# charlesq34/pointnet2

Measured on AMD Instinct MI355X. Metric: point-clouds/sec for SA(FPS+ball+group) B=32 N=4096→1024 nsample=32, higher is better.
Workload: dtype f32

## Files before the change

pointnet2_amd/csrc/fps_batch_body.h:

```cpp
#pragma once
#include "fps_pruned_body.h"

namespace pn2 {

constexpr int kBtCand = PN2_WAVE;
constexpr int kBtMaxW = 8;
#ifndef PN2_BT_UT
#define PN2_BT_UT 512
#endif
constexpr int kBtUT = PN2_BT_UT;
constexpr int kBtT = kBtUT + PN2_WAVE;
constexpr unsigned kBtEnd = 0x100u, kBtFill = 0x200u, kBtCountMask = 0xffu;

struct BtXchg {
    double list[kBtCand];
    unsigned cnt[kBtMaxW];
    unsigned bound[kBtMaxW];
    unsigned count;
    unsigned single;
    unsigned theta, vlast;
    unsigned pad[4];
};
static_assert(sizeof(BtXchg) % 16 == 0, "16-byte rows");

__host__ __device__ constexpr size_t fps_batch_xchg_offset(int P, int UT = kBtUT) { return (fps_pruned_lds_bytes(P, UT) + 15) & ~(size_t)15; }
__host__ __device__ constexpr size_t fps_batch_lds_bytes(int P, int UT = kBtUT) { return fps_batch_xchg_offset(P, UT) + 2 * sizeof(BtXchg) + 16 * kBtCand; }

__device__ __forceinline__ float vmax_f32(float a, float b)
{
    float r;
    asm("v_max_f32 %0, %1, %2" : "=v"(r) : "v"(a), "v"(b));
    return r;
}
__device__ __forceinline__ float vmed3_f32(float a, float b, float c)
{
    float r;
    asm("v_med3_f32 %0, %1, %2, %3" : "=v"(r) : "v"(a), "v"(b), "v"(c));
    return r;
}

__device__ __forceinline__ int bt_wave_max_i32_lane63(int v)
{
#define PN2_BT_STEP(ctrl) v = max(v, __builtin_amdgcn_update_dpp(0, v, ctrl, 0xf, 0xf, true))
    PN2_BT_STEP(0xB1);
    PN2_BT_STEP(0x4E);
    PN2_BT_STEP(0x141);
    PN2_BT_STEP(0x140);
    PN2_BT_STEP(0x142);
    PN2_BT_STEP(0x143);
#undef PN2_BT_STEP
    return v;
}

__device__ __forceinline__ void lds_max_u32(unsigned *p, unsigned v)
{
    asm volatile("ds_max_u32 %0, %1" :: "v"((unsigned)(size_t)p), "v"(v) : "memory");
}

inline bool fps_batch_covers(int ranks) { return ranks > 512 && ranks <= 8192; }
#ifdef PN2_BT_LAB_NEVER_AUTO
inline bool fps_batch_pays(int, int) { return false; }
#else
inline bool fps_batch_pays(int ranks, int m) { return fps_batch_covers(ranks) && m >= 256; }
#endif

#ifdef PN2_BT_STATS
__device__ unsigned long long g_bt_stats[16];
#ifndef PN2_BT_STATS_FROM
#define PN2_BT_STATS_FROM 0
#endif
#define PN2_BT_STAT(i, v) do { if (lane == 0 && cloud == 0 && j >= PN2_BT_STATS_FROM) atomicAdd(&g_bt_stats[i], (unsigned long long)(v)); } while (0)
#define PN2_BT_CLOCK() __builtin_readcyclecounter()
#else
#define PN2_BT_STAT(i, v) do { } while (0)
#define PN2_BT_CLOCK() 0ll
#pragma clang diagnostic ignored "-Wunused-variable"
#endif

#ifndef PN2_BT_LIST_HI
#define PN2_BT_LIST_HI 36
#define PN2_BT_LIST_LO 20
#endif
#ifndef PN2_BT_EARLY
#define PN2_BT_EARLY 48
#endif
#ifndef PN2_BT_ASM_LOOP
#define PN2_BT_ASM_LOOP 1
#endif
#ifndef PN2_BT_G0
#define PN2_BT_G0 0.10f
#endif
#ifndef PN2_BT_PACKED_FROM
#define PN2_BT_PACKED_FROM 16
#endif
#ifndef PN2_BT_SLOW_MIN
#define PN2_BT_SLOW_MIN 3
#define PN2_BT_QUICK 1
#define PN2_BT_SINGLE0 16
#define PN2_BT_SINGLE1 512
#endif

template <int P, int GS, bool PUBLISH, int UT = kBtUT>
__device__ __forceinline__ void fps_batch_body(int n, int m, int Q, int cloud, const float *__restrict__ xyz,
                                               int *__restrict__ out, float *__restrict__ out_xyz,
                                               unsigned long long *__restrict__ tagged, char *smem, unsigned tag = 1u)
{
    constexpr int W = UT / PN2_WAVE, NS = UT * P;
    constexpr int GW = P / GS;
    constexpr int CAP = kBtCand / W;
    constexpr int BT = UT + PN2_WAVE;
    static_assert((W * GW == 32 && (W == 4 || W == 8)) || (W == 8 && (GW == 2 || GW == 1)),
                  "32 groups on four or eight updater waves; 16 / 8 groups (2048 / 1024 rank slots) on eight");
    float4 *lds_rank = reinterpret_cast<float4 *>(smem + 256);
    BtXchg *xch = reinterpret_cast<BtXchg *>(smem + fps_batch_xchg_offset(P, UT));
    float4 *ring = reinterpret_cast<float4 *>(smem + fps_batch_xchg_offset(P, UT) + 2 * sizeof(BtXchg));

    const float *__restrict__ src = xyz + (size_t)cloud * n * 3;
    int *__restrict__ dst = out + (size_t)cloud * m;
    float *__restrict__ dxyz = out_xyz ? out_xyz + (size_t)cloud * m * 3 : nullptr;
    pn2_gu64 *gtag = PUBLISH ? (pn2_gu64 *)(tagged + (size_t)cloud * m) : nullptr;
    const int t = threadIdx.x;
    const int lane = t & 63;
    const int w = __builtin_amdgcn_readfirstlane(t >> 6);

    int j = 1;
    const int jE = min(PN2_BT_EARLY, m);
    int fill_k = -1;

    if (w == W) {
#ifndef PN2_NO_SETPRIO
        __builtin_amdgcn_s_setprio(3);
#endif
        for (int i = lane; i < (int)(2 * sizeof(BtXchg) / 4); i += PN2_WAVE) reinterpret_cast<unsigned *>(xch)[i] = 0u;
        for (int i = 0; i < kPrPrologueBarriers; ++i) __syncthreads();
        long long e0 = 0;
        for (; j < jE; ++j) {
            if (j == 8) e0 = (long long)__builtin_readcyclecounter();
            __syncthreads();
        }
        const float round_cyc = jE >= 24 ? (float)((long long)__builtin_readcyclecounter() - e0) / (float)(jE - 8) : 1e30f;
        float bt_cyc = 0.f, bt_smp = 0.f;
        int bt_n = 0, bt_paid = 0, run = PN2_BT_SINGLE0, a_prev = 0, single_next = 0;
        long long qb = 0;
        float g = PN2_BT_G0;
        int par = 0;
        if (j < m)
        for (;;) {
            const long long q0 = PN2_BT_CLOCK();
            {
                const long long qn = (long long)__builtin_readcyclecounter();
                if (bt_n > 0) {
                    bt_cyc = 0.75f * bt_cyc + (float)(qn - qb); bt_smp = 0.75f * bt_smp + (float)a_prev;
                    if (bt_n > PN2_BT_QUICK) {
                        if (bt_cyc > bt_smp * round_cyc * (bt_n > PN2_BT_SLOW_MIN ? 1.0f : 1.5f)) {
                            single_next = run;
                            run = min(2 * run, PN2_BT_SINGLE1);
                            bt_n = -1; bt_paid = 0; bt_cyc = 0.f; bt_smp = 0.f;
                        } else if (++bt_paid >= 8) {
                            run = PN2_BT_SINGLE0;
                        }
                    }
                }
                qb = qn;
                ++bt_n;
            }
            __syncthreads();
            const long long q1 = PN2_BT_CLOCK();
            BtXchg &X = xch[par];
            if (lane == 0) __hip_atomic_store(&xch[par ^ 1].count, 0u, __ATOMIC_RELAXED, __HIP_MEMORY_SCOPE_WORKGROUP);
            const uint4 c4 = *reinterpret_cast<const uint4 *>(X.cnt), c5 = *reinterpret_cast<const uint4 *>(X.cnt + 4);
            const uint4 b4 = *reinterpret_cast<const uint4 *>(X.bound), b5 = *reinterpret_cast<const uint4 *>(X.bound + 4);
            const double key = X.list[lane];
            const unsigned cw = X.cnt[lane / CAP];
            const bool valid = (unsigned)(lane & (CAP - 1)) < cw;
            const unsigned lowc = valid ? (unsigned)__double2loint(key) : 0u;
            typedef float bt_f4 __attribute__((ext_vector_type(4)));
            const bt_f4 cand = *reinterpret_cast<const bt_f4 *>(&lds_rank[lowc]);
            const int boundb = __builtin_amdgcn_readfirstlane((int)max(max(max(b4.x, b4.y), max(b4.z, b4.w)), max(max(b5.x, b5.y), max(b5.z, b5.w))));
            const int total = __builtin_amdgcn_readfirstlane((int)(c4.x + c4.y + c4.z + c4.w + c5.x + c5.y + c5.z + c5.w));
            int cval = valid ? __double2hiint(key) : (int)0xBF800000;
            const int clo = (int)lowc;
            int a = 0;
            int vlastb = 0;
            bool fill = false;
            const unsigned ring_base = (unsigned)(size_t)ring, count_addr = (unsigned)(size_t)&X.count;
            const long long q2 = PN2_BT_CLOCK();
            int bh;
            unsigned long long eq;
            auto argmax = [&]() __attribute__((always_inline)) {
                bh = __builtin_amdgcn_readlane(bt_wave_max_i32_lane63(cval), 63);
                eq = __ballot(cval == bh);
                if (__popcll(eq) != 1) {
                    PN2_BT_STAT(11, 1);
                    const double kq = cval == bh ? __hiloint2double(cval, clo) : -1.0;
                    const double km = wave_max_f64_lane63(kq);
                    const int ml = __builtin_amdgcn_readlane(__double2loint(km), 63);
                    eq = __ballot(cval == bh && clo == ml);
                    eq &= 0ull - eq;
                }
            };
            argmax();
            const int amax = min(m - j, kBtCand);
            unsigned raddr = ring_base, na = 1u;
#if PN2_BT_ASM_LOOP
            const float cx = cand.x, cy = cand.y, cz = cand.z;
            for (;;) {
                int reason, t_wl, t_sx, t_sy, t_sz, t_ms, t_cnt;
                int v_t;
                float v_dx, v_dy, v_dz;
                asm volatile(
                    "s_branch 1f\n\t"
                    "0:\n\t"
                    "s_mov_b32 %[bh], %[ms]\n\t"
                    "1:\n\t"
                    "s_mov_b64 exec, %[eq]\n\t"
                    "ds_write_b128 %[raddr], %[cand]\n\t"
                    "ds_write_b32 %[caddr], %[na]\n\t"
                    "v_mov_b32 %[cval], 0xbf800000\n\t"
                    "s_mov_b64 exec, -1\n\t"
                    "s_ff1_i32_b64 %[wl], %[eq]\n\t"
                    "s_add_i32 %[a], %[a], 1\n\t"
                    "v_add_u32 %[raddr], 16, %[raddr]\n\t"
                    "v_add_u32 %[na], 1, %[na]\n\t"
                    "s_cmp_ge_i32 %[a], %[amax]\n\t"
                    "s_cbranch_scc1 2f\n\t"
                    "v_readlane_b32 %[sx], %[cx], %[wl]\n\t"
                    "v_readlane_b32 %[sy], %[cy], %[wl]\n\t"
                    "v_max_i32_dpp %[t], %[cval], %[cval] quad_perm:[1,0,3,2] row_mask:0xf bank_mask:0xf bound_ctrl:0\n\t"
                    "v_readlane_b32 %[sz], %[cz], %[wl]\n\t"
                    "v_subrev_f32 %[dx], %[sx], %[cx]\n\t"
                    "v_max_i32_dpp %[t], %[t], %[t] quad_perm:[2,3,0,1] row_mask:0xf bank_mask:0xf bound_ctrl:0\n\t"
                    "v_subrev_f32 %[dy], %[sy], %[cy]\n\t"
                    "v_subrev_f32 %[dz], %[sz], %[cz]\n\t"
                    "v_max_i32_dpp %[t], %[t], %[t] row_half_mirror row_mask:0xf bank_mask:0xf bound_ctrl:0\n\t"
                    "v_mul_f32 %[dx], %[dx], %[dx]\n\t"
                    "v_mul_f32 %[dy], %[dy], %[dy]\n\t"
                    "v_max_i32_dpp %[t], %[t], %[t] row_mirror row_mask:0xf bank_mask:0xf bound_ctrl:0\n\t"
                    "v_mul_f32 %[dz], %[dz], %[dz]\n\t"
                    "v_add_f32 %[dx], %[dx], %[dy]\n\t"
                    "v_max_i32_dpp %[t], %[t], %[t] row_bcast:15 row_mask:0xf bank_mask:0xf bound_ctrl:0\n\t"
                    "v_add_f32 %[dx], %[dx], %[dz]\n\t"
                    "s_nop 0\n\t"
                    "v_max_i32_dpp %[t], %[t], %[t] row_bcast:31 row_mask:0xf bank_mask:0xf bound_ctrl:0\n\t"
                    "v_min_f32 %[cval], %[dx], %[cval]\n\t"
                    "s_nop 0\n\t"
                    "v_readlane_b32 %[ms], %[t], 63\n\t"
                    "s_nop 0\n\t"
                    "s_cmp_lt_i32 %[ms], %[bound]\n\t"
                    "s_cbranch_scc1 3f\n\t"
                    "v_cmp_eq_u32_e64 %[eq], %[ms], %[cval]\n\t"
                    "s_bcnt1_i32_b64 %[cnt], %[eq]\n\t"
                    "s_cmp_eq_u32 %[cnt], 1\n\t"
                    "s_cbranch_scc1 0b\n\t"
                    "s_mov_b32 %[reason], 2\n\t"
                    "s_branch 4f\n\t"
                    "2:\n\t"
                    "s_mov_b32 %[reason], 0\n\t"
                    "s_branch 4f\n\t"
                    "3:\n\t"
                    "s_mov_b32 %[reason], 1\n\t"
                    "4:"
                    : [cval] "+v"(cval), [raddr] "+v"(raddr), [na] "+v"(na), [eq] "+s"(eq), [a] "+s"(a), [bh] "+s"(bh),
                      [reason] "=&s"(reason), [wl] "=&s"(t_wl), [sx] "=&s"(t_sx), [sy] "=&s"(t_sy), [sz] "=&s"(t_sz), [ms] "=&s"(t_ms), [cnt] "=&s"(t_cnt),
                      [t] "=&v"(v_t), [dx] "=&v"(v_dx), [dy] "=&v"(v_dy), [dz] "=&v"(v_dz)
                    : [cand] "v"(cand), [caddr] "v"(count_addr), [cx] "v"(cx), [cy] "v"(cy), [cz] "v"(cz), [amax] "s"(amax), [bound] "s"(boundb)
                    : "memory", "scc");
                vlastb = bh;
                if (reason != 2) break;
                PN2_BT_STAT(12, 1);
                argmax();
                if (bh < boundb) break;
            }
#else
            for (;;) {
                asm volatile("s_mov_b64 exec, %1\n\t"
                             "ds_write_b128 %2, %3\n\t"
                             "ds_write_b32 %4, %5\n\t"
                             "v_mov_b32 %0, 0xbf800000\n\t"
                             "s_mov_b64 exec, -1"
                             : "+v"(cval) : "s"(eq), "v"(raddr), "v"(cand), "v"(count_addr), "v"(na) : "memory");
                const int wl = (int)__builtin_ctzll(eq);
                raddr += 16u; na += 1u;
                a = __builtin_amdgcn_readfirstlane(a + 1);
                vlastb = bh;
                if (a >= amax) break;
                const int ms = __builtin_amdgcn_readlane(bt_wave_max_i32_lane63(cval), 63);
                const float sx = __int_as_float(__builtin_amdgcn_readlane(__float_as_int(cand.x), wl));
                const float sy = __int_as_float(__builtin_amdgcn_readlane(__float_as_int(cand.y), wl));
                const float sz = __int_as_float(__builtin_amdgcn_readlane(__float_as_int(cand.z), wl));
                const float d = sqdist(cand.x, cand.y, cand.z, sx, sy, sz);
                cval = __float_as_int(vmin_f32(d, __int_as_float(cval)));
                if (ms < boundb) break;
                eq = __ballot(cval == ms);
                bh = ms;
                if (__popcll(eq) != 1) {
                    PN2_BT_STAT(12, 1);
                    argmax();
                    if (bh < boundb) break;
                }
            }
#endif
            if (vlastb == 0) { fill = true; fill_k = __builtin_amdgcn_readlane(__float_as_int(cand.w), (int)__builtin_ctzll(eq)); }
            const long long q3 = PN2_BT_CLOCK();
            if (total > PN2_BT_LIST_HI) g = fmaxf(g * 0.8f, 1.0f / 128.0f);
            else if (total < PN2_BT_LIST_LO) g = fminf(g * 1.25f, 0.5f);
            X.theta = __float_as_uint(__fmul_rn(__int_as_float(vlastb), 1.0f - g));
            X.vlast = (unsigned)vlastb;
            a_prev = a;
            int single = min(single_next, m - (j + a));
            if (single_next) { PN2_BT_STAT(13, single); PN2_BT_STAT(14, 1); }
            single_next = 0;
            single = __builtin_amdgcn_readfirstlane(single);
            X.single = (unsigned)single;
            if (lane == 0)
                __hip_atomic_store(&X.count, (unsigned)a | kBtEnd | (fill ? kBtFill : 0u), __ATOMIC_RELEASE, __HIP_MEMORY_SCOPE_WORKGROUP);
            PN2_BT_STAT(0, 1); PN2_BT_STAT(1, a); PN2_BT_STAT(4, total); PN2_BT_STAT(6, q2 - q1); PN2_BT_STAT(7, q3 - q2); PN2_BT_STAT(8, q1 - q0);
            j = __builtin_amdgcn_readfirstlane(j + a);
            if (fill || j >= m) break;
            for (int i = 0; i < single; ++i) __syncthreads();
            j += single;
            if (j >= m) break;
            par ^= 1;
        }
    } else {
        PrSlots<P> S;
        fps_pruned_prologue<P, GS, UT>(n, Q, src, smem, S);
        pn2_f2 (&xx)[P / 2] = S.xx;
        pn2_f2 (&yy)[P / 2] = S.yy;
        pn2_f2 (&zz)[P / 2] = S.zz;
        float (&md)[P] = S.md;
        unsigned (&low)[P] = S.low;
        float blx, bly, blz, bhx, bhy, bhz;
        {
            const float *gbox = reinterpret_cast<const float *>(smem + 256 + (size_t)16 * NS + (size_t)kPrHistRows * kPrBins * 4);
            const float *o = gbox + (w * GW + (lane & (GW - 1))) * 8;
            blx = o[0]; bly = o[1]; blz = o[2]; bhx = o[4]; bhy = o[5]; bhz = o[6];
        }
        pn2_f2 sxy = {0.f, 0.f}, syy = {0.f, 0.f}, szk = {0.f, 0.f};
        auto update_group = [&](auto gic) __attribute__((always_inline)) {
            constexpr int gi = decltype(gic)::value;
            constexpr int H = GS / 2;
            pn2_f2 dx[H], dy[H], dz[H];
#pragma unroll
            for (int h = 0; h < H; ++h) dx[h] = pk_sub_bcast_lo(xx[gi * H + h], sxy);
#pragma unroll
            for (int h = 0; h < H; ++h) dy[h] = pk_sub_bcast_lo(yy[gi * H + h], syy);
#pragma unroll
            for (int h = 0; h < H; ++h) dz[h] = pk_sub_bcast_lo(zz[gi * H + h], szk);
#pragma unroll
            for (int h = 0; h < H; ++h) dx[h] = pk_mul(dx[h], dx[h]);
#pragma unroll
            for (int h = 0; h < H; ++h) dy[h] = pk_mul(dy[h], dy[h]);
#pragma unroll
            for (int h = 0; h < H; ++h) dz[h] = pk_mul(dz[h], dz[h]);
#pragma unroll
            for (int h = 0; h < H; ++h) dx[h] = pk_add(dx[h], dy[h]);
#pragma unroll
            for (int h = 0; h < H; ++h) dx[h] = pk_add(dx[h], dz[h]);
#pragma unroll
            for (int h = 0; h < H; ++h) {
                const int p0 = gi * GS + 2 * h;
                md[p0] = vmin_f32(dx[h].x, md[p0]);
                md[p0 + 1] = vmin_f32(dx[h].y, md[p0 + 1]);
            }
        };
        auto update_all = [&]() __attribute__((always_inline)) {
            update_group(std::integral_constant<int, 0>());
            if constexpr (GW >= 2) update_group(std::integral_constant<int, 1>());
            if constexpr (GW >= 4) { update_group(std::integral_constant<int, 2>()); update_group(std::integral_constant<int, 3>()); }
            if constexpr (GW == 8) {
                update_group(std::integral_constant<int, 4>()); update_group(std::integral_constant<int, 5>());
                update_group(std::integral_constant<int, 6>()); update_group(std::integral_constant<int, 7>());
            }
        };
        {
            const float4 s = lds_rank[NS - 1];
            sxy.x = s.x; syy.x = s.y; szk.x = s.z;
            update_all();
        }
        if (t == 0) {
            dst[0] = 0;
            if (PUBLISH) __hip_atomic_store(gtag, (unsigned long long)tag << 32, __ATOMIC_RELAXED, __HIP_MEMORY_SCOPE_AGENT);
        }
        unsigned vlastb = __float_as_uint(1e38f);
        unsigned thetab = __float_as_uint(1e38f);
        auto single_rounds = [&](const int jend) __attribute__((always_inline)) {
            double *partial = reinterpret_cast<double *>(smem);
            for (; j < jend; ++j) {
                double kd[P];
#pragma unroll
                for (int p = 0; p < P; ++p) kd[p] = __hiloint2double(__float_as_int(md[p]), (int)low[p]);
#pragma unroll
                for (int st = 1; st < P; st <<= 1)
#pragma unroll
                    for (int i = 0; i + st < P; i += 2 * st)
                        asm("v_max_f64 %0, %1, %2" : "=v"(kd[i]) : "v"(kd[i]), "v"(kd[i + st]));
                const double wd = wave_max_f64_lane63(kd[0]);
                double *slot = partial + (j & 1) * W;
                if (lane == 63) slot[w] = wd;
                __syncthreads();
                double key[W];
#pragma unroll
                for (int i = 0; i < W; ++i) key[i] = slot[i];
#pragma unroll
                for (int st = 1; st < W; st <<= 1)
#pragma unroll
                    for (int i = 0; i + st < W; i += 2 * st)
                        asm("v_max_f64 %0, %1, %2" : "=v"(key[i]) : "v"(key[i]), "v"(key[i + st]));
                vlastb = (unsigned)__double2hiint(key[0]);
                const float4 s = lds_rank[(unsigned)__double2loint(key[0])];
                if (t == 0) {
                    const int k = __float_as_int(s.w);
                    dst[j] = k;
                    if (PUBLISH)
                        __hip_atomic_store(gtag + j, ((unsigned long long)tag << 32) | (unsigned long long)(unsigned)k, __ATOMIC_RELAXED,
                                           __HIP_MEMORY_SCOPE_AGENT);
                }
                if constexpr (P >= PN2_BT_PACKED_FROM) {
                    sxy.x = s.x; syy.x = s.y; szk.x = s.z;
                    update_all();
                } else {
#pragma unroll
                    for (int p = 0; p < P; ++p) {
                        const float d = p & 1 ? sqdist(xx[p / 2].y, yy[p / 2].y, zz[p / 2].y, s.x, s.y, s.z)
                                              : sqdist(xx[p / 2].x, yy[p / 2].x, zz[p / 2].x, s.x, s.y, s.z);
                        md[p] = vmin_f32(d, md[p]);
                    }
                }
            }
            thetab = __float_as_uint(__fmul_rn(__uint_as_float(vlastb), 1.0f - PN2_BT_G0));
        };
        if (jE > 1) single_rounds(jE);
        int par = 0;
        if (j < m)
        for (;;) {
            BtXchg &X = xch[par];
            const long long u0 = PN2_BT_CLOCK();
            double kl;
            float sec;
            {
                double kd[P];
                float hv[P / 2], lv[P / 2];
#pragma unroll
                for (int p = 0; p < P; ++p) kd[p] = __hiloint2double(__float_as_int(md[p]), (int)low[p]);
#pragma unroll
                for (int i = 0; i < P / 2; ++i) { hv[i] = vmax_f32(md[2 * i], md[2 * i + 1]); lv[i] = vmin_f32(md[2 * i], md[2 * i + 1]); }
#pragma unroll
                for (int st = 1; st < P; st <<= 1)
#pragma unroll
                    for (int i = 0; i + st < P; i += 2 * st)
                        asm("v_max_f64 %0, %1, %2" : "=v"(kd[i]) : "v"(kd[i]), "v"(kd[i + st]));
#pragma unroll
                for (int st = 1; st < P / 2; st <<= 1)
#pragma unroll
                    for (int i = 0; i + st < P / 2; i += 2 * st) {
                        const float ll = vmax_f32(lv[i], lv[i + st]);
                        lv[i] = vmed3_f32(hv[i], hv[i + st], ll);
                        hv[i] = vmax_f32(hv[i], hv[i + st]);
                    }
                kl = kd[0];
                sec = lv[0];
            }
            const unsigned vb = (unsigned)__double2hiint(kl);
            unsigned long long mask = __ballot(vb >= thetab);
            int cnt = __popcll(mask);
            unsigned thb = thetab;
            bool exact = false;
            if (cnt > CAP) {
                unsigned lob = thetab, hib = vlastb + 1u;
                for (int it = 0; it < 16; ++it) {
                    const unsigned mid = lob + ((hib - lob) >> 1);
                    if (mid == lob) break;
                    const unsigned long long mk = __ballot(vb >= mid);
                    const int c = __popcll(mk);
                    PN2_BT_STAT(3, 1);
                    if (c > CAP) lob = mid;
                    else if (c == 0) hib = mid;
                    else { mask = mk; cnt = c; thb = mid; break; }
                }
                exact = cnt > CAP;
            } else if (cnt == 0) {
                exact = true;
            }
            if (exact) {
                PN2_BT_STAT(2, 1);
                const double wk = wave_max_f64_lane63(kl);
                const int bh = __builtin_amdgcn_readlane(__double2hiint(wk), 63), bl = __builtin_amdgcn_readlane(__double2loint(wk), 63);
                unsigned long long mk = __ballot(__double2hiint(kl) == bh && __double2loint(kl) == bl);
                mk &= 0ull - mk;
                if (cnt != 0) thb = (unsigned)bh + 1u;
                mask = mk;
                cnt = 1;
            }
            if ((mask >> lane) & 1ull) {
                const int pos = __builtin_amdgcn_mbcnt_hi((unsigned)(mask >> 32), __builtin_amdgcn_mbcnt_lo((unsigned)mask, 0u));
                X.list[w * CAP + pos] = kl;
                lds_max_u32(&X.bound[w], __float_as_uint(sec) + 1u);
            }
            if (lane == 0) {
                X.cnt[w] = (unsigned)cnt;
                lds_max_u32(&X.bound[w], thb);
            }
            const long long u1 = PN2_BT_CLOCK();
            asm volatile("s_waitcnt lgkmcnt(0)" ::: "memory");
            __syncthreads();
            const long long u2 = PN2_BT_CLOCK();
            if (lane == 0) xch[par ^ 1].bound[w] = 0u;
            int done = 0;
            unsigned c;
            const float thr = __fadd_rn(__fmul_rn(__uint_as_float(vlastb), 1.00001f), 1e-30f);
            for (;;) {
                c = __hip_atomic_load(&X.count, __ATOMIC_ACQUIRE, __HIP_MEMORY_SCOPE_WORKGROUP);
                c = (unsigned)__builtin_amdgcn_readfirstlane((int)c);
                const int avail = (int)(c & kBtCountMask);
                if (avail == done) {
                    if (c & kBtEnd) break;
                    __builtin_amdgcn_s_sleep(1);
                    continue;
                }
                constexpr int CH = PN2_WAVE / GW;
                constexpr unsigned long long kStride = GW == 8 ? 0x0101010101010101ull : GW == 4 ? 0x1111111111111111ull
                                                       : GW == 2 ? 0x5555555555555555ull : ~0ull;
                const int np = min(avail - done, CH);
                const int pi = lane / GW;
                const float4 s = ring[done + (pi < np ? pi : 0)];
                const float ax = __fsub_rn(s.x, __builtin_amdgcn_fmed3f(s.x, blx, bhx));
                const float ay = __fsub_rn(s.y, __builtin_amdgcn_fmed3f(s.y, bly, bhy));
                const float az = __fsub_rn(s.z, __builtin_amdgcn_fmed3f(s.z, blz, bhz));
                const float bd = __fadd_rn(__fadd_rn(__fmul_rn(ax, ax), __fmul_rn(ay, ay)), __fmul_rn(az, az));
                unsigned long long touched = ~__ballot(bd >= thr);
                if (np * GW < 64) touched &= (1ull << (np * GW)) - 1ull;
                if (touched) {
                    if (2 * __popcll(touched) >= GW * np) {
                        for (int p = 0; p < np; ++p) {
                            sxy.x = __int_as_float(__builtin_amdgcn_readlane(__float_as_int(s.x), p * GW));
                            syy.x = __int_as_float(__builtin_amdgcn_readlane(__float_as_int(s.y), p * GW));
                            szk.x = __int_as_float(__builtin_amdgcn_readlane(__float_as_int(s.z), p * GW));
                            update_all();
                        }
                    } else {
                        auto one_group = [&](auto gic) __attribute__((always_inline)) {
                            constexpr int g8 = decltype(gic)::value;
                            unsigned long long mg = touched & (kStride << g8);
                            while (mg) {
                                const int sl = (int)__builtin_ctzll(mg) & ~(GW - 1);
                                mg &= mg - 1ull;
                                sxy.x = __int_as_float(__builtin_amdgcn_readlane(__float_as_int(s.x), sl));
                                syy.x = __int_as_float(__builtin_amdgcn_readlane(__float_as_int(s.y), sl));
                                szk.x = __int_as_float(__builtin_amdgcn_readlane(__float_as_int(s.z), sl));
                                PN2_BT_STAT(5, 1);
                                update_group(gic);
                            }
                        };
                        one_group(std::integral_constant<int, 0>());
                        if constexpr (GW >= 2) one_group(std::integral_constant<int, 1>());
                        if constexpr (GW >= 4) { one_group(std::integral_constant<int, 2>()); one_group(std::integral_constant<int, 3>()); }
                        if constexpr (GW == 8) {
                            one_group(std::integral_constant<int, 4>()); one_group(std::integral_constant<int, 5>());
                            one_group(std::integral_constant<int, 6>()); one_group(std::integral_constant<int, 7>());
                        }
                    }
                }
                done += np;
            }
            const long long u3 = PN2_BT_CLOCK();
            if (w == 0) { PN2_BT_STAT(9, u1 - u0); PN2_BT_STAT(10, u3 - u2); }
            const int a = (int)(c & kBtCountMask);
            if (w == 0 && lane < a) {
                const int k = __float_as_int(ring[lane].w);
                dst[j + lane] = k;
                if (PUBLISH)
                    __hip_atomic_store(gtag + (j + lane), ((unsigned long long)tag << 32) | (unsigned long long)(unsigned)k, __ATOMIC_RELAXED,
                                       __HIP_MEMORY_SCOPE_AGENT);
            }
            if (c & kBtFill) fill_k = __float_as_int(ring[a - 1].w);
            j += a;
            if ((c & kBtFill) || j >= m) break;
            thetab = X.theta;
            vlastb = X.vlast;
            const int single = __builtin_amdgcn_readfirstlane((int)X.single);
            if (single) {
                single_rounds(min(j + single, m));
                if (j >= m) break;
            }
            par ^= 1;
        }
    }
    if (fill_k >= 0) {
        for (int i = j + t; i < m; i += BT) {
            dst[i] = fill_k;
            if (PUBLISH)
                __hip_atomic_store(gtag + i, ((unsigned long long)tag << 32) | (unsigned long long)(unsigned)fill_k, __ATOMIC_RELAXED,
                                   __HIP_MEMORY_SCOPE_AGENT);
        }
    }
    fps_gather_epilogue<BT>(m, src, dst, dxyz);
}

}
```

Before: 141,400.

## Speculatively compute per-lane FPS keys while waiting and carry candidate rows in exchange

Two changes to the batched FPS round. Each lane's candidate row (coordinates) is now written into the exchange buffer next to its key, so the argmax wave can read it directly instead of doing an indirect lds_rank lookup. Waves that would otherwise sleep while polling the ring now recompute their per-lane max keys speculatively, and reuse them next round if no further updates arrived. This hides the key-reduction latency behind the wait, at the cost of a larger exchange struct in LDS and wasted work when more updates arrive.

```diff
diff --git a/pointnet2_amd/csrc/fps_batch_body.h b/pointnet2_amd/csrc/fps_batch_body.h
--- a/pointnet2_amd/csrc/fps_batch_body.h
+++ b/pointnet2_amd/csrc/fps_batch_body.h
@@ -12,7 +12,17 @@
 constexpr int kBtT = kBtUT + PN2_WAVE;
 constexpr unsigned kBtEnd = 0x100u, kBtFill = 0x200u, kBtCountMask = 0xffu;
 
+#ifndef PN2_BT_LIST_ROWS
+#define PN2_BT_LIST_ROWS 1
+#endif
+#ifndef PN2_BT_SPEC_KEYS
+#define PN2_BT_SPEC_KEYS 1
+#endif
+
 struct BtXchg {
+#if PN2_BT_LIST_ROWS
+    float4 row[kBtCand];
+#endif
     double list[kBtCand];
     unsigned cnt[kBtMaxW];
     unsigned bound[kBtMaxW];
@@ -172,10 +182,16 @@
             const uint4 b4 = *reinterpret_cast<const uint4 *>(X.bound), b5 = *reinterpret_cast<const uint4 *>(X.bound + 4);
             const double key = X.list[lane];
             const unsigned cw = X.cnt[lane / CAP];
+            typedef float bt_f4 __attribute__((ext_vector_type(4)));
+#if PN2_BT_LIST_ROWS
+            const bt_f4 cand = *reinterpret_cast<const bt_f4 *>(&X.row[lane]);
             const bool valid = (unsigned)(lane & (CAP - 1)) < cw;
             const unsigned lowc = valid ? (unsigned)__double2loint(key) : 0u;
-            typedef float bt_f4 __attribute__((ext_vector_type(4)));
+#else
+            const bool valid = (unsigned)(lane & (CAP - 1)) < cw;
+            const unsigned lowc = valid ? (unsigned)__double2loint(key) : 0u;
             const bt_f4 cand = *reinterpret_cast<const bt_f4 *>(&lds_rank[lowc]);
+#endif
             const int boundb = __builtin_amdgcn_readfirstlane((int)max(max(max(b4.x, b4.y), max(b4.z, b4.w)), max(max(b5.x, b5.y), max(b5.z, b5.w))));
             const int total = __builtin_amdgcn_readfirstlane((int)(c4.x + c4.y + c4.z + c4.w + c5.x + c5.y + c5.z + c5.w));
             int cval = valid ? __double2hiint(key) : (int)0xBF800000;
@@ -430,37 +446,44 @@
             }
             thetab = __float_as_uint(__fmul_rn(__uint_as_float(vlastb), 1.0f - PN2_BT_G0));
         };
+        double kl = 0.0;
+        float sec = 0.f;
+        float4 krow = {0.f, 0.f, 0.f, 0.f};
+        bool keyed = false;
+        auto lane_keys = [&]() __attribute__((always_inline)) {
+            double kd[P];
+            float hv[P / 2], lv[P / 2];
+#pragma unroll
+            for (int p = 0; p < P; ++p) kd[p] = __hiloint2double(__float_as_int(md[p]), (int)low[p]);
+#pragma unroll
+            for (int i = 0; i < P / 2; ++i) { hv[i] = vmax_f32(md[2 * i], md[2 * i + 1]); lv[i] = vmin_f32(md[2 * i], md[2 * i + 1]); }
+#pragma unroll
+            for (int st = 1; st < P; st <<= 1)
+#pragma unroll
+                for (int i = 0; i + st < P; i += 2 * st)
+                    asm("v_max_f64 %0, %1, %2" : "=v"(kd[i]) : "v"(kd[i]), "v"(kd[i + st]));
+#pragma unroll
+            for (int st = 1; st < P / 2; st <<= 1)
+#pragma unroll
+                for (int i = 0; i + st < P / 2; i += 2 * st) {
+                    const float ll = vmax_f32(lv[i], lv[i + st]);
+                    lv[i] = vmed3_f32(hv[i], hv[i + st], ll);
+                    hv[i] = vmax_f32(hv[i], hv[i + st]);
+                }
+            kl = kd[0];
+            sec = lv[0];
+#if PN2_BT_LIST_ROWS
+            krow = lds_rank[(unsigned)__double2loint(kl)];
+#endif
+        };
         if (jE > 1) single_rounds(jE);
         int par = 0;
         if (j < m)
         for (;;) {
             BtXchg &X = xch[par];
             const long long u0 = PN2_BT_CLOCK();
-            double kl;
-            float sec;
-            {
-                double kd[P];
-                float hv[P / 2], lv[P / 2];
-#pragma unroll
-                for (int p = 0; p < P; ++p) kd[p] = __hiloint2double(__float_as_int(md[p]), (int)low[p]);
-#pragma unroll
-                for (int i = 0; i < P / 2; ++i) { hv[i] = vmax_f32(md[2 * i], md[2 * i + 1]); lv[i] = vmin_f32(md[2 * i], md[2 * i + 1]); }
-#pragma unroll
-                for (int st = 1; st < P; st <<= 1)
-#pragma unroll
-                    for (int i = 0; i + st < P; i += 2 * st)
-                        asm("v_max_f64 %0, %1, %2" : "=v"(kd[i]) : "v"(kd[i]), "v"(kd[i + st]));
-#pragma unroll
-                for (int st = 1; st < P / 2; st <<= 1)
-#pragma unroll
-                    for (int i = 0; i + st < P / 2; i += 2 * st) {
-                        const float ll = vmax_f32(lv[i], lv[i + st]);
-                        lv[i] = vmed3_f32(hv[i], hv[i + st], ll);
-                        hv[i] = vmax_f32(hv[i], hv[i + st]);
-                    }
-                kl = kd[0];
-                sec = lv[0];
-            }
+            if (!keyed) lane_keys();
+            if (w == 0) PN2_BT_STAT(15, keyed ? 1 : 0);
             const unsigned vb = (unsigned)__double2hiint(kl);
             unsigned long long mask = __ballot(vb >= thetab);
             int cnt = __popcll(mask);
@@ -495,6 +518,9 @@
             if ((mask >> lane) & 1ull) {
                 const int pos = __builtin_amdgcn_mbcnt_hi((unsigned)(mask >> 32), __builtin_amdgcn_mbcnt_lo((unsigned)mask, 0u));
                 X.list[w * CAP + pos] = kl;
+#if PN2_BT_LIST_ROWS
+                X.row[w * CAP + pos] = krow;
+#endif
                 lds_max_u32(&X.bound[w], __float_as_uint(sec) + 1u);
             }
             if (lane == 0) {
@@ -507,6 +533,7 @@
             const long long u2 = PN2_BT_CLOCK();
             if (lane == 0) xch[par ^ 1].bound[w] = 0u;
             int done = 0;
+            int keyed_at = 0;
             unsigned c;
             const float thr = __fadd_rn(__fmul_rn(__uint_as_float(vlastb), 1.00001f), 1e-30f);
             for (;;) {
@@ -515,7 +542,12 @@
                 const int avail = (int)(c & kBtCountMask);
                 if (avail == done) {
                     if (c & kBtEnd) break;
-                    __builtin_amdgcn_s_sleep(1);
+                    if (PN2_BT_SPEC_KEYS && P <= 8 && keyed_at != done) {
+                        lane_keys();
+                        keyed_at = done;
+                    } else {
+                        __builtin_amdgcn_s_sleep(1);
+                    }
                     continue;
                 }
                 constexpr int CH = PN2_WAVE / GW;
@@ -566,6 +598,7 @@
             const long long u3 = PN2_BT_CLOCK();
             if (w == 0) { PN2_BT_STAT(9, u1 - u0); PN2_BT_STAT(10, u3 - u2); }
             const int a = (int)(c & kBtCountMask);
+            keyed = keyed_at == done;
             if (w == 0 && lane < a) {
                 const int k = __float_as_int(ring[lane].w);
                 dst[j + lane] = k;
@@ -581,6 +614,7 @@
             const int single = __builtin_amdgcn_readfirstlane((int)X.single);
             if (single) {
                 single_rounds(min(j + single, m));
+                keyed = false;
                 if (j >= m) break;
             }
             par ^= 1;
```

Measured after the change: 141,900, median of 6. No clear change (+0.4%).
